# lucidrains/transfusion-pytorch

Hardware: NVIDIA H100
Metric: train tokens/sec (text+latent) at d=512 L=8 seq=1024 (higher is better)
Workload: dtype bf16

## Files before the change

### include/tfx_b200.h

```cpp
#ifndef TFX_B200_H
#define TFX_B200_H

#ifdef __cplusplus
extern "C" {
#endif

#define TFX_B200_VERSION 200

const char* tfx_last_error(void);
int tfx_version(void);
int tfx_init(int device);


int tfx_gemm_set_cluster_mode(int mode);

int tfx_gemm_store(const void* A, long long lda, int a_mn_major, const void* B, long long ldb, int b_mn_major, int M, int N, int K,
                   float* out_f32, long long ld_f32, void* out_bf16, long long ld_bf16, const float* bias, const long long* row_off,
                   float alpha, int accumulate, int k_splits, void* stream);

int tfx_gemm_qkvg(const void* u, long long ldu, const void* W, long long ldw, int M, int H, int D, void* q, void* k, void* v, float* gates, float* qk_inv,
                  const float* q_gamma, const float* k_gamma, const int* rope_pos, const float* rope_cs_t , int rope_len,
                  const int* kv_rows, float* mix_pre, void* stream);

int tfx_gemm_resid(const void* A, long long lda, const void* A2, long long lda2, int K1, const void* W, long long ldw, int M, int N, int K, const float* bias,
                   const float* x_res, float* x_out, void* x_out_bf16, void* y_bf16, const int* cond_row, const float* zgate, long long zgate_ld,
                   const float* layerscale, void* stream);

int tfx_gemm_geglu(const void* u, long long ldu, const void* W1p, long long ldw, const float* b1p, int M, int Np, int K, void* vg, void* h, void* stream);
int tfx_gemm_geglu_drop(const void* u, long long ldu, const void* W1p, long long ldw, const float* b1p, int M, int Np, int K, void* vg, void* h,
                        const void* drop_key , float p, int layer, void* stream);

int tfx_attn_fwd(const void* q, const void* k, const void* v, long long ld_q, long long ld_k, long long ld_v, const float* gates, int H,
                 const int* kv_limit, const int* tile_q0, const int* tile_qend, const int* tile_kv0, const int* tile_kvend, int n_tiles,
                 void* o, long long ld_o, float* lse, int M, float scale, float softcap, const float* skip_if_fast , void* stream);
int tfx_attn_fast_params(const float* q_gamma, const float* k_gamma, int dim_head, float scale, float softcap, float* params , void* stream);
int tfx_attn_fwd_tc(const void* q, const void* k, const void* v, long long ld_q, long long ld_k, long long ld_v, const float* gates, int H,
                    const int* kv_limit, const int* tile_q0, const int* tile_qend, const int* tile_kv0, const int* tile_kvend, int n_tiles,
// ... 106 lines not shown
```

### transfusion_pytorch_b200/_lib.py

```python
from __future__ import annotations

import ctypes
import os
from ctypes import c_void_p, c_int, c_longlong, c_ulonglong, c_float, c_char_p, POINTER

_HERE = os.path.dirname(os.path.abspath(__file__))
LIB_PATH = os.path.join(_HERE, 'libtfx_b200.so')

_lib = None

VP, I, LL, F, ULL = c_void_p, c_int, c_longlong, c_float, c_ulonglong

SIGNATURES = {
    'tfx_init': [I],
    'tfx_gemm_set_cluster_mode': [I],
    'tfx_gemm_store': [VP, LL, I, VP, LL, I, I, I, I, VP, LL, VP, LL, VP, VP, F, I, I, VP],
    'tfx_gemm_qkvg': [VP, LL, VP, LL, I, I, I, VP, VP, VP, VP, VP, VP, VP, VP, VP, I, VP, VP, VP],
    'tfx_gemm_resid': [VP, LL, VP, LL, I, VP, LL, I, I, I, VP, VP, VP, VP, VP, VP, VP, LL, VP, VP],
    'tfx_gemm_geglu': [VP, LL, VP, LL, VP, I, I, I, VP, VP, VP],
    'tfx_gemm_geglu_drop': [VP, LL, VP, LL, VP, I, I, I, VP, VP, VP, F, I, VP],
    'tfx_attn_fwd': [VP, VP, VP, LL, LL, LL, VP, I, VP, VP, VP, VP, VP, I, VP, LL, VP, I, F, F, VP, VP],
    'tfx_attn_fwd_tc': [VP, VP, VP, LL, LL, LL, VP, I, VP, VP, VP, VP, VP, I, VP, LL, VP, I, I, F, F, VP, VP],
    'tfx_attn_fast_params': [VP, VP, I, F, F, VP, VP],
    'tfx_attn_bwd_prep': [VP, VP, VP, VP, VP, VP, VP, I, I, VP],
    'tfx_attn_bwd': [VP, VP, VP, VP, LL, LL, LL, LL, VP, VP, VP, VP, VP, VP, VP, I, VP, VP, VP, LL, I, I, F, F, VP, VP],
    'tfx_attn_bwd_tc': [VP, VP, VP, VP, LL, LL, LL, LL, VP, VP, VP, VP, VP, VP, VP, VP, I, VP, VP, VP, LL, I, I, F, F, VP, VP],
    'tfx_qk_bwd_pack': [VP, VP, VP, VP, VP, VP, VP, VP, VP, VP, VP, VP, LL, VP, VP, I, I, VP],
    'tfx_adaln_fwd': [VP, VP, VP, LL, VP, VP, VP, I, I, VP],
    'tfx_adaln_bwd': [VP, VP, VP, VP, VP, LL, VP, VP, VP, LL, VP, I, I, VP],
    'tfx_resid_bwd': [VP, VP, VP, VP, LL, VP, VP, VP, LL, VP, VP, I, I, VP],
    'tfx_attn_residual_fwd': [VP, I, VP, VP, VP, VP, VP, I, I, VP],
    'tfx_attn_residual_bwd': [VP, VP, I, VP, VP, VP, VP, VP, VP, VP, VP, I, I, I, VP],
    'tfx_attn_residual_bwd2': [VP, I, I, VP, VP, VP, VP, I, VP, VP, VP, VP, VP, I, VP, VP, VP, I, I, VP],
    'tfx_attn_residual_fwd_h16': [VP, I, VP, VP, VP, VP, VP, I, I, VP],
    'tfx_attn_residual_bwd_h16': [VP, VP, I, VP, VP, VP, VP, VP, VP, VP, VP, I, I, I, VP],
    'tfx_rmsnorm_fwd': [VP, VP, VP, VP, VP, VP, I, I, VP],
    'tfx_rmsnorm_bwd': [VP, VP, VP, VP, VP, I, I, VP],
    'tfx_rep_cos_fwd_bwd': [VP, VP, I, VP, I, VP, VP, VP, VP, I, I, VP],
# ... 61 lines not shown
    lib.tfx_last_error.argtypes = []
    lib.tfx_version.restype = c_int
    lib.tfx_version.argtypes = []
    lib.tfx_geglu_bwd_rows_per_block.restype = c_int
    lib.tfx_geglu_bwd_rows_per_block.argtypes = []
    lib.tfx_attn_residual_bwd_workspace_floats.restype = c_longlong
    lib.tfx_attn_residual_bwd_workspace_floats.argtypes = [c_int, c_int]
    lib.tfx_rep_cos_blocks.restype = c_int
    lib.tfx_rep_cos_blocks.argtypes = [c_int]
    for name, argtypes in SIGNATURES.items():
        fn = getattr(lib, name)
        fn.argtypes = argtypes
        fn.restype = c_int
    _lib = lib
    return lib


def check(rc: int, name: str):
    if rc != 0:
        msg = _lib.tfx_last_error().decode(errors = 'replace') if _lib is not None else ''
        raise TfxError(f'{name} failed (code {rc}): {msg}')


class Ops:

    def __init__(self):
        self.lib = load()
        import torch
        self._torch = torch
        self.launches = 0
        self.timing = None
        self.order = None

    def stream(self):
        return self._torch.cuda.current_stream().cuda_stream

    def __getattr__(self, name):
        fn = getattr(self.lib, 'tfx_' + name)
        torch = self._torch

        def call(*args):
            conv = []
            for a in args:
                if a is None:
                    conv.append(None)
                elif torch.is_tensor(a):
# ... 20 lines not shown
```

### transfusion_pytorch_b200/csrc/gemm_api.cu

```cuda
#include "gemm_sm90.cuh"
#include "common.cuh"
#include "../../include/tfx_b200.h"
#include <string.h>

namespace tfx { int num_sms(); }
using namespace tfx;
#define ST(s) reinterpret_cast<cudaStream_t>(s)

static int finish(int rc, const char* what) {
  if (rc == 0) return 0;
  if (rc <= -1000) set_error("%s: cuTensorMapEncodeTiled failed (CUresult %d) - check 16-byte alignment of pointers and row pitches", what, -(rc + 1000));
  else if (rc == -1) set_error("%s: cuTensorMapEncodeTiled entry point unavailable (no CUDA driver?)", what);
  else if (rc == -2) set_error("%s: cudaFuncSetAttribute(max dynamic smem) failed: %s", what, cudaGetErrorString(cudaGetLastError()));
  else set_error("%s: kernel launch failed: %s", what, cudaGetErrorString(cudaGetLastError()));
  return rc;
}

static int dispatch_major(const GemmOperand& A, const GemmOperand& B, const GemmParams& p, cudaStream_t st) {
  const int sms = num_sms();
  if (!A.mn_major && !B.mn_major) return launch_gemm_t<false, false, EPI_STORE>(A, B, p, sms, st);
  if (!A.mn_major && B.mn_major) return launch_gemm_t<false, true, EPI_STORE>(A, B, p, sms, st);
  if (A.mn_major && B.mn_major) return launch_gemm_t<true, true, EPI_STORE>(A, B, p, sms, st);
  return launch_gemm_t<true, false, EPI_STORE>(A, B, p, sms, st);
}

extern "C" {

int tfx_gemm_set_cluster_mode(int mode) {
  TFX_REQUIRE(mode >= 1 && mode <= 3, "gemm_set_cluster_mode: mode %d not in {1 (never pair, default), 2 (always pair), 3 (pair long-K launches)}", mode);
  gemm_cluster_mode_ref() = mode;
  return 0;
}

int tfx_gemm_store(const void* A, long long lda, int a_mn_major, const void* B, long long ldb, int b_mn_major, int M, int N, int K,
                   float* out_f32, long long ld_f32, void* out_bf16, long long ld_bf16, const float* bias, const long long* row_off,
                   float alpha, int accumulate, int k_splits, void* stream) {
  if (M <= 0 || N <= 0) return 0;
  TFX_REQUIRE(K > 0, "gemm_store: K must be > 0");
  TFX_REQUIRE(lda % 8 == 0 && ldb % 8 == 0, "gemm_store: operand row pitches (%lld, %lld) must be multiples of 8 bf16", lda, ldb);
  TFX_REQUIRE(!(k_splits > 1) || (accumulate && out_f32 && !out_bf16 && !bias), "gemm_store: split-K requires fp32 accumulate output only");
  GemmParams p; memset(&p, 0, sizeof(p));
  p.M = M; p.N = N; p.K = K; p.k_splits = k_splits < 1 ? 1 : k_splits;
  p.out_f32 = out_f32; p.ld_f32 = ld_f32; p.out_bf16 = (__nv_bfloat16*)out_bf16; p.ld_bf16 = ld_bf16; p.bias = bias; p.row_off = row_off;
  p.alpha = alpha; p.accumulate_f32 = accumulate;
  GemmOperand a{A, lda, a_mn_major != 0}, b{B, ldb, b_mn_major != 0};
  const int rc = dispatch_major(a, b, p, ST(stream));
  return finish(rc, "gemm_store");
}

int tfx_gemm_qkvg(const void* u, long long ldu, const void* W, long long ldw, int M, int H, int D, void* q, void* k, void* v, float* gates, float* qk_inv,
                  const float* q_gamma, const float* k_gamma, const int* rope_pos, const float* rope_cs_t, int rope_len, const int* kv_rows, float* mix_pre, void* stream) {
  if (M <= 0) return 0;
  TFX_REQUIRE(!mix_pre || H <= 16, "gemm_qkvg: the value-residual mix columns share the 32-column gate slab: heads must be <= 16 (got %d)", H);
// ... 48 lines not shown
```

### transfusion_pytorch_b200/csrc/gemm_sm90.cuh

```cuda
#pragma once
#include "sm90_ptx.cuh"
#include "dropout.cuh"

namespace tfx {

constexpr int GEMM_BM = 128;
constexpr int GEMM_BN = 128;
constexpr int GEMM_BK = 64;
constexpr int GEMM_UK = 16;

enum : int { EPI_STORE = 0, EPI_QKVG = 1, EPI_RESID = 2, EPI_GEGLU = 3, EPI_GEGLU_DROP = 4 };

struct GemmParams {
  int M, N, K;
  int k_splits;
  float* out_f32; long long ld_f32;
  __nv_bfloat16* out_bf16; long long ld_bf16;
  const float* bias;
  const long long* row_off;
  float alpha;
  int accumulate_f32;
  int K1;
  int H;
  __nv_bfloat16 *q, *k, *v;
// ... 133 lines not shown
      *reinterpret_cast<uint4*>(g + row * pitch + ch * 16) = *reinterpret_cast<const uint4*>(sw + row * 64 + ((ch ^ ((row >> 1) & 3)) << 4));
  }
}

__device__ __forceinline__ void stg64_store_rows(const uint8_t* sw, int lane, uint8_t* g, long long pitch, int rows_valid, const int* __restrict__ rows) {
#pragma unroll
  for (int it = 0; it < 4; ++it) {
    const int row = it * 8 + (lane >> 2), ch = lane & 3;
    if (row < rows_valid)
      *reinterpret_cast<uint4*>(g + (long long)rows[row] * pitch + ch * 16) = *reinterpret_cast<const uint4*>(sw + row * 64 + ((ch ^ ((row >> 1) & 3)) << 4));
  }
}
template <int CH>
__device__ __forceinline__ void stg_store_rows(const uint8_t* sw, int lane, uint8_t* g, long long pitch, int rows_valid, const int* __restrict__ rows) {
  constexpr int RPI = 32 / CH;
#pragma unroll
  for (int it = 0; it < 32 / RPI; ++it) {
    const int row = it * RPI + lane / CH, ch = lane % CH;
    if (row < rows_valid)
      *reinterpret_cast<uint4*>(g + (long long)rows[row] * pitch + ch * 16) = *reinterpret_cast<const uint4*>(sw + row * 128 + ((ch ^ (row & 7)) << 4));
  }
}

template <bool A_MN, bool B_MN, int EPI, int CL>
__global__ void __launch_bounds__(384, 1)
gemm_sm90_kernel(const __grid_constant__ CUtensorMap tmA, const __grid_constant__ CUtensorMap tmA2, const __grid_constant__ CUtensorMap tmB, const GemmParams p) {
  using Cfg = GemmCfg<EPI>;
  constexpr bool GEGLU = EPI == EPI_GEGLU || EPI == EPI_GEGLU_DROP;
  constexpr int BN = GEMM_BN;
  constexpr int STAGES = Cfg::STAGES;
  static_assert(Cfg::STAGE_BYTES % 1024 == 0 && 2 * STAGES <= 32, "stage alignment / barrier area");
  extern __shared__ __align__(1024) uint8_t smem_raw[];
  uint8_t* smem = smem_raw;
  if (threadIdx.x == 0 && (smem_u32(smem) & 1023u) != 0) __trap();
  uint8_t* acc = smem + STAGES * Cfg::STAGE_BYTES;
  uint8_t* staging = acc + Cfg::ACC_BYTES;
  uint64_t* bars = reinterpret_cast<uint64_t*>(staging + Cfg::STAGING);
  uint64_t* full_bar = bars;
  uint64_t* empty_bar = bars + STAGES;

  const int warp = threadIdx.x >> 5, lane = threadIdx.x & 31;
  const int m_tiles = (p.M + GEMM_BM - 1) / GEMM_BM;
  const int n_tiles = (p.N + BN - 1) / BN;
  const int kb_total = (p.K + GEMM_BK - 1) / GEMM_BK;
  const int kb_per_split = (kb_total + p.k_splits - 1) / p.k_splits;
  const int m_units = (m_tiles + CL - 1) / CL;
// ... 119 lines not shown
      {
        const int r0 = quad * 16 + (lane >> 2);
#pragma unroll
        for (int q = 0; q < 16; ++q) {
          const int c = 8 * q + 2 * (lane & 3);
          *reinterpret_cast<float2*>(acc + acc_off(r0, c)) = make_float2(d0[4 * q], d0[4 * q + 1]);
          *reinterpret_cast<float2*>(acc + acc_off(r0 + 8, c)) = make_float2(d0[4 * q + 2], d0[4 * q + 3]);
          *reinterpret_cast<float2*>(acc + acc_off(r0 + 64, c)) = make_float2(d1[4 * q], d1[4 * q + 1]);
          *reinterpret_cast<float2*>(acc + acc_off(r0 + 72, c)) = make_float2(d1[4 * q + 2], d1[4 * q + 3]);
        }
      }
      named_bar_sync(BAR_TILE + cw, 128);

      const int wrow0 = m_blk * GEMM_BM + quad * 32;
      const int row = wrow0 + lane;
      const bool row_ok = row < p.M;
      const int rows_valid = min(32, p.M - wrow0);
      const int col0 = n_blk * BN;
      int qk_pos = 0;
      if constexpr (EPI == EPI_QKVG) { qk_pos = row_ok ? p.rope_pos[row] : 0; }
      if constexpr (EPI == EPI_RESID) { qk_pos = (row_ok && p.cond_row) ? p.cond_row[row] : -1; }

      if constexpr (EPI == EPI_STORE) {
        const bool f32_staged = p.out_f32 && (p.row_off || (p.ld_f32 & 3) == 0) && ((reinterpret_cast<uintptr_t>(p.out_f32) & 15) == 0);
        const bool bf16_staged = p.out_bf16 && (p.ld_bf16 & 7) == 0 && ((reinterpret_cast<uintptr_t>(p.out_bf16) & 15) == 0);
#pragma unroll 1
        for (int c = 0; c < BN / 32; ++c) {
          const int cbase = col0 + c * 32;
          if (cbase >= p.N) break;
          uint32_t r[32];
          acc_ld32(acc, erow, c * 32, r);
          const bool full = cbase + 32 <= p.N;
          float v[32];
#pragma unroll
          for (int j = 0; j < 32; ++j) v[j] = __uint_as_float(r[j]);
          if (p.alpha != 1.f) {
#pragma unroll
            for (int j = 0; j < 32; ++j) v[j] *= p.alpha;
          }
          if (p.bias) {
            if (full) {
#pragma unroll
              for (int j = 0; j < 32; j += 4) { const float4 b = *reinterpret_cast<const float4*>(p.bias + cbase + j); v[j] += b.x; v[j + 1] += b.y; v[j + 2] += b.z; v[j + 3] += b.w; }
            } else {
              for (int j = 0; j < 32; ++j) if (cbase + j < p.N) v[j] += p.bias[cbase + j];
            }
          }
          if (p.out_f32) {
            if (full && f32_staged) {
#pragma unroll
              for (int j = 0; j < 32; ++j) r[j] = __float_as_uint(v[j]);
              stg_put<8>(sw, lane, r);
              __syncwarp();
#pragma unroll
              for (int it = 0; it < 8; ++it) {
                const int rr = it * 4 + (lane >> 3), ch = lane & 7;
                if (rr < rows_valid) {
                  const long long off = p.row_off ? p.row_off[wrow0 + rr] : (long long)(wrow0 + rr) * p.ld_f32;
                  if (off >= 0) {
                    float* dst = p.out_f32 + off + cbase + ch * 4;
                    const float4 t = *reinterpret_cast<const float4*>(sw + rr * 128 + ((ch ^ (rr & 7)) << 4));
                    if ((reinterpret_cast<uintptr_t>(dst) & 15) == 0) {
                      if (p.accumulate_f32) asm volatile("red.global.add.v4.f32 [%0], {%1, %2, %3, %4};" ::"l"(dst), "f"(t.x), "f"(t.y), "f"(t.z), "f"(t.w) : "memory");
                      else *reinterpret_cast<float4*>(dst) = t;
                    } else {
                      if (p.accumulate_f32) { atomicAdd(dst, t.x); atomicAdd(dst + 1, t.y); atomicAdd(dst + 2, t.z); atomicAdd(dst + 3, t.w); }
                      else { dst[0] = t.x; dst[1] = t.y; dst[2] = t.z; dst[3] = t.w; }
                    }
                  }
                }
              }
              __syncwarp();
            } else if (row_ok) {
              const long long off = p.row_off ? p.row_off[row] : (long long)row * p.ld_f32;
              if (off >= 0) {
                float* dst = p.out_f32 + off + cbase;
                for (int j = 0; j < 32; ++j)
                  if (cbase + j < p.N) { if (p.accumulate_f32) atomicAdd(dst + j, v[j]); else dst[j] = v[j]; }
              }
            }
          }
          if (p.out_bf16) {
            if (full && bf16_staged) {
              uint32_t w[16];
#pragma unroll
              for (int j = 0; j < 16; ++j) w[j] = pack_bf16(v[2 * j], v[2 * j + 1]);
              stg_put<4>(sw, lane, w);
              __syncwarp();
              stg_store<4>(sw, lane, reinterpret_cast<uint8_t*>(p.out_bf16 + (long long)wrow0 * p.ld_bf16 + cbase), p.ld_bf16 * 2, rows_valid);
              __syncwarp();
            } else if (row_ok) {
              __nv_bfloat16* dst = p.out_bf16 + (long long)row * p.ld_bf16 + cbase;
              for (int j = 0; j < 32; ++j) if (cbase + j < p.N) dst[j] = __float2bfloat16(v[j]);
            }
          }
        }
      } else if constexpr (EPI == EPI_QKVG) {
        const int tps = p.H >> 1;
        const int kind = n_blk / tps;
        const int tis = n_blk - kind * tps;
        const long long HI = (long long)p.H * 64;
        if (kind <= 1) {
          const float* gamma = kind == 0 ? p.q_gamma : p.k_gamma;
          __nv_bfloat16* dstm = kind == 0 ? p.q : p.k;
          const float2* cs = p.rope_cs + qk_pos;
#pragma unroll
          for (int hh = 0; hh < 2; ++hh) {
            uint32_t r0[32], r1[32];
            acc_ld32(acc, erow, hh * 64, r0);
            acc_ld32(acc, erow, hh * 64 + 32, r1);
            float ss = 0.f;
#pragma unroll
            for (int j = 0; j < 32; ++j) { float a = __uint_as_float(r0[j]), b = __uint_as_float(r1[j]); ss += a * a + b * b; }
            const float inv = 1.f / fmaxf(sqrtf(ss), 1e-12f);
            const int head = tis * 2 + hh;
            if (row_ok) p.qk_inv[(long long)row * 2 * p.H + kind * p.H + head] = inv;
            const float sc = inv * 8.f;
            uint32_t outw[32];
// ... 152 lines not shown
            const float2 o = geglu_pair(make_float2(g[j], g[j + 1]), make_float2(v[j], v[j + 1]));
            g[j] = o.x; g[j + 1] = o.y;
          }
          if constexpr (EPI == EPI_GEGLU_DROP) {
#pragma unroll
            for (int j = 0; j < 32; ++j) g[j] = (keep[c] >> j) & 1u ? g[j] * p.drop.scale : 0.f;
          }
          __syncwarp();
          stg64_put_pack(sw, lane, g);
          __syncwarp();
          stg64_store(sw, lane, reinterpret_cast<uint8_t*>(p.h + (long long)wrow0 * (p.N / 2) + n_blk * 64 + c * 32), (long long)p.N, rows_valid);
          __syncwarp();
        }
      }
      if (!GEGLU && has_next) named_bar_arrive(BAR_ACC + (cw ^ 1), 256);
    }
  }
  if constexpr (CL > 1) {
    __syncthreads();
    cluster_sync_all();
  }
}

typedef CUresult (*PFN_encodeTiled)(CUtensorMap*, CUtensorMapDataType, cuuint32_t, void*, const cuuint64_t*, const cuuint64_t*,
                                    const cuuint32_t*, const cuuint32_t*, CUtensorMapInterleave, CUtensorMapSwizzle,
                                    CUtensorMapL2promotion, CUtensorMapFloatOOBfill);

inline PFN_encodeTiled get_encode_fn() {
  static PFN_encodeTiled fn = nullptr;
  if (!fn) {
    void* f = nullptr;
    cudaDriverEntryPointQueryResult qres;
    if (cudaGetDriverEntryPoint("cuTensorMapEncodeTiled", &f, cudaEnableDefault, &qres) != cudaSuccess || !f) return nullptr;
    fn = reinterpret_cast<PFN_encodeTiled>(f);
  }
  return fn;
}

inline int make_tmap_bf16(CUtensorMap* tm, const void* ptr, long long inner, long long outer, long long ld, int box_rows) {
  PFN_encodeTiled enc = get_encode_fn();
  if (!enc) return -1;
  cuuint64_t dims[2] = {(cuuint64_t)inner, (cuuint64_t)outer};
  cuuint64_t strides[1] = {(cuuint64_t)ld * 2};
  cuuint32_t box[2] = {64, (cuuint32_t)box_rows};
  cuuint32_t estr[2] = {1, 1};
  CUresult r = enc(tm, CU_TENSOR_MAP_DATA_TYPE_BFLOAT16, 2, const_cast<void*>(ptr), dims, strides, box, estr,
                   CU_TENSOR_MAP_INTERLEAVE_NONE, CU_TENSOR_MAP_SWIZZLE_128B, CU_TENSOR_MAP_L2_PROMOTION_L2_256B,
                   CU_TENSOR_MAP_FLOAT_OOB_FILL_NONE);
  return r == CUDA_SUCCESS ? 0 : -(int)r - 1000;
}

struct GemmOperand {
  const void* ptr;
  long long ld;
  bool mn_major;
  const void* ptr2 = nullptr;
  long long ld2 = 0;
};

inline int& gemm_cluster_mode_ref() {
  static int mode = -1;
  if (mode < 0) { const char* e = getenv("TFX_GEMM_CLUSTER"); mode = e ? atoi(e) : 1; }
  return mode;
}

template <bool A_MN, bool B_MN, int EPI>
int launch_gemm_t(const GemmOperand& A, const GemmOperand& B, const GemmParams& p_in, int num_sms, cudaStream_t stream) {
  using Cfg = GemmCfg<EPI>;
  GemmParams p = p_in;
  CUtensorMap tmA, tmA2, tmB;
  int rc;
  const bool two = (!A_MN) && A.ptr2 != nullptr;
  if (!two) p.K1 = p.K;
  if (!A_MN) rc = make_tmap_bf16(&tmA, A.ptr, two ? p.K1 : p.K, p.M, A.ld, GEMM_BM); else rc = make_tmap_bf16(&tmA, A.ptr, p.M, p.K, A.ld, GEMM_BK);
  if (rc) return rc;
  if (two) { rc = make_tmap_bf16(&tmA2, A.ptr2, p.K - p.K1, p.M, A.ld2, GEMM_BM); if (rc) return rc; } else tmA2 = tmA;
  {
    const int kbt = (p.K + GEMM_BK - 1) / GEMM_BK;
    if (p.k_splits < 1) p.k_splits = 1;
    if (p.k_splits > kbt) p.k_splits = kbt;
    const int per = (kbt + p.k_splits - 1) / p.k_splits;
    p.k_splits = (kbt + per - 1) / per;
  }
  const int m_tiles = (p.M + GEMM_BM - 1) / GEMM_BM, n_tiles = (p.N + GEMM_BN - 1) / GEMM_BN;
  const int items = m_tiles * n_tiles * p.k_splits;
  if (items <= 0) return 0;
  const int mode = gemm_cluster_mode_ref();
  const int kb_item = ((p.K + GEMM_BK - 1) / GEMM_BK + p.k_splits - 1) / p.k_splits;
  const bool paired = mode == 2 || (mode == 3 && m_tiles >= 2 && kb_item >= 16 && items >= 2 * num_sms);
  if (!B_MN) rc = make_tmap_bf16(&tmB, B.ptr, p.K, p.N, B.ld, paired ? GEMM_BN / 2 : GEMM_BN); else rc = make_tmap_bf16(&tmB, B.ptr, p.N, p.K, B.ld, GEMM_BK);
  if (rc) return rc;
  if (paired) {
    auto kern = gemm_sm90_kernel<A_MN, B_MN, EPI, 2>;
    static int max_clusters = 0;
    cudaLaunchConfig_t cfg;
    memset(&cfg, 0, sizeof(cfg));
    cudaLaunchAttribute at[1];
    at[0].id = cudaLaunchAttributeClusterDimension;
    at[0].val.clusterDim.x = 2; at[0].val.clusterDim.y = 1; at[0].val.clusterDim.z = 1;
    cfg.blockDim = dim3(Cfg::THREADS); cfg.dynamicSmemBytes = Cfg::SMEM_BYTES; cfg.stream = stream; cfg.attrs = at; cfg.numAttrs = 1;
    if (!max_clusters) {
      if (cudaFuncSetAttribute(kern, cudaFuncAttributeMaxDynamicSharedMemorySize, Cfg::SMEM_BYTES) != cudaSuccess) return -2;
      cfg.gridDim = dim3(2 * (num_sms / 2));
      int nc = 0;
      if (cudaOccupancyMaxActiveClusters(&nc, kern, &cfg) != cudaSuccess || nc < 1) { cudaGetLastError(); nc = num_sms / 2; }
      max_clusters = nc < num_sms / 2 ? nc : num_sms / 2;
    }
    const int pair_items = ((m_tiles + 1) / 2) * n_tiles * p.k_splits;
    const int clusters = pair_items < max_clusters ? pair_items : max_clusters;
    cfg.gridDim = dim3(2 * clusters);
    return cudaLaunchKernelEx(&cfg, kern, tmA, tmA2, tmB, p) == cudaSuccess ? 0 : -3;
// ... 14 lines not shown
```

### transfusion_pytorch_b200/engine.py

```python
from __future__ import annotations

import math
import os
import ctypes
from dataclasses import dataclass

import numpy as np
import torch
from torch import Tensor

from . import _lib
from ._pinned import POOL
from .modality_processing import RaggedBatch

BF16, F32, I32, I64 = torch.bfloat16, torch.float32, torch.int32, torch.int64


def _round_up(x: int, m: int) -> int:
    return (x + m - 1) // m * m


_EMPTY_I32 = np.zeros(0, dtype = np.int32)


# ... 30 lines not shown
    tab = np.zeros(len(jobs), dtype = dt)
    blk_job, blk_first = [], []
    for j, (src, ld_src, c_src, row_src, d, r_dst, c_dst, f32) in enumerate(jobs):
        tab[j] = (src.data_ptr(), ld_src, row_src.data_ptr() if row_src is not None else 0, d.data_ptr(), r_dst, c_src, c_dst, f32, 0)
        nb = (r_dst * c_dst + 2047) // 2048
        blk_first.append(len(blk_job))
        blk_job.extend([j] * nb)
    return (torch.from_numpy(tab.view(np.uint8).copy()).to(device), torch.tensor(blk_job, dtype = I32, device = device),
            torch.tensor(blk_first, dtype = I32, device = device), len(blk_job))


def w1_row_src(inner: int) -> np.ndarray:
    Ip = _round_up(inner, 64)
    src = np.full(2 * Ip, -1, dtype = np.int64)
    for t in range(Ip // 64):
        for j in range(64):
            c = 64 * t + j
            if c < inner:
                src[128 * t + j] = c
                src[128 * t + 64 + j] = inner + c
    return src


def wgrad_splits(n_out, n_in, K, sms, ks):
    tiles = ((n_out + 127) // 128) * ((n_in + 255) // 256 if (n_in % 256 == 0 or n_in >= 1024) else (n_in + 127) // 128)
    best, best_eff = 1, 0.0
    for s in range(1, 65):
        if K // s < 1024 and s > 1:
            break
        items = tiles * s
        eff = items / (-(-items // sms) * sms)
        if eff > best_eff + 0.02 or (abs(eff - best_eff) <= 0.02 and s <= ks and s > best):
            best, best_eff = s, eff
    return best


class KVCache:

    def __init__(self, engine, n_slabs: int, cap: int):
        self.n_slabs, self.cap, self.rows = int(n_slabs), int(cap), int(n_slabs) * int(cap)
        nbytes = 2 * engine.depth * self.rows * engine.HI * 2
        assert nbytes < 96 << 30, f'kv cache of {nbytes / 2**30:.1f} GiB requested ({n_slabs} slabs x {cap} rows): lower max_length / batch the prompts'
        self.k = torch.zeros(engine.depth, self.rows, engine.HI, device = engine.device, dtype = BF16)
        self.v = torch.zeros(engine.depth, self.rows, engine.HI, device = engine.device, dtype = BF16)
        self.vl = torch.zeros_like(self.v) if engine.laser else None

    def slab_start(self, s):
        return np.asarray(s, dtype = np.int64) * self.cap


class Engine:
    def __init__(self, model):
        self.ops = _lib.Ops()
        self.model = model
        tr = model.transformer
        self.D, self.H, self.depth = tr.dim, tr.heads, tr.depth
        self.HI = self.H * 64
# ... 563 lines not shown
        st = self.state
        assert st['train'], 'backward() needs a train forward'
        rep_at = None
        if g_rep is not None:
            rep_at = st.get('rep_layer')
            assert rep_at is not None and g_rep.dtype == F32 and g_rep.is_contiguous() and g_rep.shape == (st['rb'].M, self.D), 'g_rep: fp32 [M, D] of a rep_layer forward'
        self._prepare_grads()
        self._grads_clean = False
        self._dirty = True
        if gscale is not None:
            gs = gscale.detach().float().reshape(1)
            self.ops.scale_bf16(st['dlogits'], gs, st['dlogits'].numel())
            for dp in st['dpred']:
                if dp is not None:
                    self.ops.scale_bf16(dp, gs, dp.numel())
        rb, dv = st['rb'], st['rb'].dev
        o, D, HI, H, Ip, M, inner = self.ops, self.D, self.HI, self.H, self.Ip, st['rb'].M, self.inner
        pk, nc, S = self.packed, rb.n_cond, rb.S
        cond_row = dv['cond_row'] if nc > 0 else None
        tab_ld, zg_ld = self.W * 3 * D, self.W * D
        ks = max(1, min(64, M // 2048))
        sms = torch.cuda.get_device_properties(self.device).multi_processor_count
        def ksplit(n_out, n_in, K = M):
            return wgrad_splits(n_out, n_in, K, sms, ks)
        def wgrad(dy, ld_dy, n_out, act, ld_act, n_in, gname, K = M):
            o.gemm_store(dy, ld_dy, 1, act, ld_act, 1, n_out, n_in, K, self.G(gname), n_in, None, 0, None, None, 1.0, 1, ksplit(n_out, n_in, K))

        dlog = st['dlogits']
        d_out = self.buf('d_out', (M, D), F32)
        o.gemm_store(dlog, self.Vp, 0, pk['wvocab'], D, 1, M, D, self.V, d_out, D, None, 0, None, None, 1.0, 0, 1)
        wgrad(dlog, self.Vp, self.V, st['outb'], D, D, 'to_text_logits.weight')
        if S > 0:
            dmod = self.buf('dmod', (S, D), F32)
            any_flow = False
            for t, (s0, s1) in enumerate(rb.type_rows):
                n = s1 - s0
                dp = st['dpred'][t] if n else None
                if dp is None:
                    if n:
                        dmod[s0:s1].zero_()
                    continue
                any_flow = True
                dl, dlp = self.dls[t], self.dlp[t]
                o.gemm_store(dp, dlp, 0, pk[f'wm2l{t}'], D, 1, n, D, dl, dmod[s0:s1], D, None, 0, None, None, 1.0, 0, 1)
                wgrad(dp, dlp, dl, st['omod'][s0:s1], D, D, f'model_to_latent_projs.{t}.weight', K = n)
            dneg = None
            if any_flow and self.clean:
# ... 242 lines not shown
        a = eng.buf('rh_a', (M, D), F32)
        o.gemm_store(h, Ip, 0, self.w2p, Ip, 0, M, D, Ip, a, D, None, 0, b2, None, 1.0, 0, 1)
        da = eng.buf('rh_da', (M, D), BF16)
        part = eng.buf('rh_part', (int(o.lib.tfx_rep_cos_blocks(M)),), torch.float64)
        ticket = eng.buf('rh_ticket', (1,), I32, zero = True)
        loss = eng.buf('rh_loss', (1,), F32)
        o.rep_cos_fwd_bwd(a, teacher, 1 if teacher.dtype == BF16 else 0, g, M, da, part, ticket, loss, M, D)
        self.state = dict(x = x, u = u, vg = vg, h = h, da = da, g = g, M = M)
        return loss[0].clone()

    def backward(self, g_loss: Tensor | None = None) -> Tensor:
        eng, o, st = self.eng, self.eng.ops, self.state
        M, D, inner, Ip = st['M'], self.D, self.inner, self.Ip
        head = self.head
        params = [head[0].gamma, head[1].net[0].weight, head[1].net[0].bias, head[1].net[3].weight, head[1].net[3].bias]
        for p in params:
            if p.grad is None:
                p.grad = torch.zeros_like(p)
        ggamma, gw1, gb1, gw2, gb2 = (p.grad for p in params)
        da = st['da']
        if g_loss is not None:
            o.scale_bf16(da, (g_loss.detach().float().reshape(1) / st['g']), da.numel())
        sms = torch.cuda.get_device_properties(eng.device).multi_processor_count
        ks = max(1, min(64, M // 2048))
        dh = eng.buf('rh_dh', (M, Ip), BF16)
        o.gemm_store(da, D, 0, self.w2p, Ip, 1, M, Ip, D, None, 0, dh, Ip, None, None, 1.0, 0, 1)
        o.gemm_store(da, D, 1, st['h'], Ip, 1, D, inner, M, gw2, 0, None, 0, None, self.w2_rows, 1.0, 1, wgrad_splits(D, inner, M, sms, ks))
        o.colsum_bf16(da, D, M, D, None, gb2)
        dvg = eng.buf('rh_dvg', (M, 2 * Ip), BF16)
        rpb = o.lib.tfx_geglu_bwd_rows_per_block()
        nblk = (M + rpb - 1) // rpb
        part = eng.buf('rh_geglu_part', (nblk, 2 * Ip), F32)
        o.geglu_bwd(dh, st['vg'], dvg, M, Ip, None, None, part)
        o.colsum_f32(part, 2 * Ip, nblk, 2 * Ip, self.b1_cols, gb1)
        du = eng.buf('rh_du', (M, D), F32)
        o.gemm_store(dvg, 2 * Ip, 0, self.w1p, D, 1, M, D, 2 * Ip, du, D, None, 0, None, None, 1.0, 0, 1)
        o.gemm_store(dvg, 2 * Ip, 1, st['u'], D, 1, 2 * Ip, D, M, gw1, 0, None, 0, None, self.w1_rows, 1.0, 1, wgrad_splits(2 * Ip, D, M, sms, ks))
        gx = eng.buf('rh_gx', (M, D), F32)
        o.rmsnorm_bwd(du, st['x'], head[0].gamma, gx, ggamma, M, D)
        return gx
```

Before: 1.186 million.

## Add 256-row wide GEMM kernel for long-K store launches and cost-based split choice

Adds a second warp-specialized sm90 GEMM kernel using 256x128 tiles, where each consumer warpgroup issues two m64n128 wgmma per k-step. It is used for gemm_store calls whose per-item K length is at least 16 blocks, mainly the weight-gradient GEMMs. The intent is more reuse of B tiles and fewer items per tile. The k-split heuristic now queries the library for item geometry and picks the smallest split within 5% of a wave-quantized cost estimate, and it is cached. The shared store epilogue is factored into a helper, and misaligned f32 rows now take a realigned vector path. The trade-offs are fewer resident work items, which risks worse wave balance, and more register pressure from 128 accumulators per thread.

New measurement: 1.222 million, median of 6. 1.03x the previous value.

```diff
diff --git a/include/tfx_b200.h b/include/tfx_b200.h
--- a/include/tfx_b200.h
+++ b/include/tfx_b200.h
@@ -13,6 +13,10 @@
 
 
 int tfx_gemm_set_cluster_mode(int mode);
+
+int tfx_gemm_set_wide_mode(int mode);
+
+int tfx_gemm_store_items(int M, int N, int K, int a_mn_major, int b_mn_major, int k_splits, int* geometry);
 
 int tfx_gemm_store(const void* A, long long lda, int a_mn_major, const void* B, long long ldb, int b_mn_major, int M, int N, int K,
                    float* out_f32, long long ld_f32, void* out_bf16, long long ld_bf16, const float* bias, const long long* row_off,
diff --git a/transfusion_pytorch_b200/_lib.py b/transfusion_pytorch_b200/_lib.py
--- a/transfusion_pytorch_b200/_lib.py
+++ b/transfusion_pytorch_b200/_lib.py
@@ -14,6 +14,8 @@
 SIGNATURES = {
     'tfx_init': [I],
     'tfx_gemm_set_cluster_mode': [I],
+    'tfx_gemm_set_wide_mode': [I],
+    'tfx_gemm_store_items': [I, I, I, I, I, I, VP],
     'tfx_gemm_store': [VP, LL, I, VP, LL, I, I, I, I, VP, LL, VP, LL, VP, VP, F, I, I, VP],
     'tfx_gemm_qkvg': [VP, LL, VP, LL, I, I, I, VP, VP, VP, VP, VP, VP, VP, VP, VP, I, VP, VP, VP],
     'tfx_gemm_resid': [VP, LL, VP, LL, I, VP, LL, I, I, I, VP, VP, VP, VP, VP, VP, VP, LL, VP, VP],
@@ -121,6 +123,13 @@
         raise TfxError(f'{name} failed (code {rc}): {msg}')
 
 
+def gemm_store_items(M: int, N: int, K: int, a_mn: int, b_mn: int, k_splits: int):
+    lib = load()
+    geo = (c_int * 4)()
+    check(lib.tfx_gemm_store_items(M, N, K, a_mn, b_mn, k_splits, geo), 'tfx_gemm_store_items')
+    return tuple(geo)
+
+
 class Ops:
 
     def __init__(self):
diff --git a/transfusion_pytorch_b200/csrc/gemm_api.cu b/transfusion_pytorch_b200/csrc/gemm_api.cu
--- a/transfusion_pytorch_b200/csrc/gemm_api.cu
+++ b/transfusion_pytorch_b200/csrc/gemm_api.cu
@@ -18,6 +18,12 @@
 
 static int dispatch_major(const GemmOperand& A, const GemmOperand& B, const GemmParams& p, cudaStream_t st) {
   const int sms = num_sms();
+  if (gemm_store_wide(p.K, p.k_splits)) {
+    if (!A.mn_major && !B.mn_major) return launch_gemm_wide_t<false, false>(A, B, p, sms, st);
+    if (!A.mn_major && B.mn_major) return launch_gemm_wide_t<false, true>(A, B, p, sms, st);
+    if (A.mn_major && B.mn_major) return launch_gemm_wide_t<true, true>(A, B, p, sms, st);
+    return launch_gemm_wide_t<true, false>(A, B, p, sms, st);
+  }
   if (!A.mn_major && !B.mn_major) return launch_gemm_t<false, false, EPI_STORE>(A, B, p, sms, st);
   if (!A.mn_major && B.mn_major) return launch_gemm_t<false, true, EPI_STORE>(A, B, p, sms, st);
   if (A.mn_major && B.mn_major) return launch_gemm_t<true, true, EPI_STORE>(A, B, p, sms, st);
@@ -29,6 +35,24 @@
 int tfx_gemm_set_cluster_mode(int mode) {
   TFX_REQUIRE(mode >= 1 && mode <= 3, "gemm_set_cluster_mode: mode %d not in {1 (never pair, default), 2 (always pair), 3 (pair long-K launches)}", mode);
   gemm_cluster_mode_ref() = mode;
+  return 0;
+}
+
+int tfx_gemm_set_wide_mode(int mode) {
+  TFX_REQUIRE(mode >= 1 && mode <= 3, "gemm_set_wide_mode: mode %d not in {1 (long work items, default), 2 (always), 3 (never)}", mode);
+  gemm_wide_mode_ref() = mode;
+  return 0;
+}
+
+int tfx_gemm_store_items(int M, int N, int K, int a_mn_major, int b_mn_major, int k_splits, int* geometry) {
+  TFX_REQUIRE(M > 0 && N > 0 && K > 0 && geometry, "gemm_store_items: needs M, N, K > 0 (got %d, %d, %d) and an output array", M, N, K);
+  (void)a_mn_major; (void)b_mn_major;
+  const int tile_m = gemm_store_wide(K, k_splits) ? GemmWideCfg::BM : GEMM_BM;
+  const int s = gemm_effective_splits(K, k_splits);
+  geometry[0] = ((M + tile_m - 1) / tile_m) * ((N + GEMM_BN - 1) / GEMM_BN) * s;
+  geometry[1] = gemm_kb_per_item(K, s);
+  geometry[2] = tile_m;
+  geometry[3] = s;
   return 0;
 }
 
diff --git a/transfusion_pytorch_b200/csrc/gemm_sm90.cuh b/transfusion_pytorch_b200/csrc/gemm_sm90.cuh
--- a/transfusion_pytorch_b200/csrc/gemm_sm90.cuh
+++ b/transfusion_pytorch_b200/csrc/gemm_sm90.cuh
@@ -179,6 +179,99 @@
   }
 }
 
+template <class RowOf>
+__device__ __forceinline__ void store_slice(const GemmParams& p, uint8_t* sw, int lane, uint32_t (&r)[32], int cbase, RowOf row_of) {
+  const bool f32_staged = p.out_f32 && (p.row_off || (p.ld_f32 & 3) == 0) && ((reinterpret_cast<uintptr_t>(p.out_f32) & 15) == 0);
+  const bool bf16_staged = p.out_bf16 && (p.ld_bf16 & 7) == 0 && ((reinterpret_cast<uintptr_t>(p.out_bf16) & 15) == 0);
+  const int row = row_of(lane);
+  const bool row_ok = row < p.M;
+  const bool full = cbase + 32 <= p.N;
+  float v[32];
+#pragma unroll
+  for (int j = 0; j < 32; ++j) v[j] = __uint_as_float(r[j]);
+  if (p.alpha != 1.f) {
+#pragma unroll
+    for (int j = 0; j < 32; ++j) v[j] *= p.alpha;
+  }
+  if (p.bias) {
+    if (full) {
+#pragma unroll
+      for (int j = 0; j < 32; j += 4) { const float4 b = *reinterpret_cast<const float4*>(p.bias + cbase + j); v[j] += b.x; v[j + 1] += b.y; v[j + 2] += b.z; v[j + 3] += b.w; }
+    } else {
+      for (int j = 0; j < 32; ++j) if (cbase + j < p.N) v[j] += p.bias[cbase + j];
+    }
+  }
+  if (p.out_f32) {
+    if (full && f32_staged) {
+#pragma unroll
+      for (int j = 0; j < 32; ++j) r[j] = __float_as_uint(v[j]);
+      stg_put<8>(sw, lane, r);
+      __syncwarp();
+      auto put = [&](float* dst, float x) { if (p.accumulate_f32) atomicAdd(dst, x); else *dst = x; };
+#pragma unroll
+      for (int it = 0; it < 8; ++it) {
+        const int rr = it * 4 + (lane >> 3), ch = lane & 7;
+        const int grow = row_of(rr);
+        if (grow < p.M) {
+          const long long off = p.row_off ? p.row_off[grow] : (long long)grow * p.ld_f32;
+          if (off >= 0) {
+            float* drow = p.out_f32 + off + cbase;
+            const uint8_t* srow = sw + rr * 128;
+            const int a = (int)(reinterpret_cast<uintptr_t>(drow) >> 2) & 3;
+            if (a == 0) {
+              float* dst = drow + ch * 4;
+              const float4 t = *reinterpret_cast<const float4*>(srow + ((ch ^ (rr & 7)) << 4));
+              if (p.accumulate_f32) asm volatile("red.global.add.v4.f32 [%0], {%1, %2, %3, %4};" ::"l"(dst), "f"(t.x), "f"(t.y), "f"(t.z), "f"(t.w) : "memory");
+              else *reinterpret_cast<float4*>(dst) = t;
+            } else {
+              const int pe = 4 - a;
+              auto col = [&](int j) { return *reinterpret_cast<const float*>(srow + (((j >> 2) ^ (rr & 7)) << 4) + (j & 3) * 4); };
+              if (ch < 7) {
+                const int j = pe + 4 * ch;
+                float* dst = drow + j;
+                const float4 t = make_float4(col(j), col(j + 1), col(j + 2), col(j + 3));
+                if (p.accumulate_f32) asm volatile("red.global.add.v4.f32 [%0], {%1, %2, %3, %4};" ::"l"(dst), "f"(t.x), "f"(t.y), "f"(t.z), "f"(t.w) : "memory");
+                else *reinterpret_cast<float4*>(dst) = t;
+              } else {
+#pragma unroll
+                for (int i = 0; i < 4; ++i) { const int j = i < pe ? i : 28 + i; put(drow + j, col(j)); }
+              }
+            }
+          }
+        }
+      }
+      __syncwarp();
+    } else if (row_ok) {
+      const long long off = p.row_off ? p.row_off[row] : (long long)row * p.ld_f32;
+      if (off >= 0) {
+        float* dst = p.out_f32 + off + cbase;
+        for (int j = 0; j < 32; ++j)
+          if (cbase + j < p.N) { if (p.accumulate_f32) atomicAdd(dst + j, v[j]); else dst[j] = v[j]; }
+      }
+    }
+  }
+  if (p.out_bf16) {
+    if (full && bf16_staged) {
+      uint32_t w[16];
+#pragma unroll
+      for (int j = 0; j < 16; ++j) w[j] = pack_bf16(v[2 * j], v[2 * j + 1]);
+      stg_put<4>(sw, lane, w);
+      __syncwarp();
+#pragma unroll
+      for (int it = 0; it < 4; ++it) {
+        const int rr = it * 8 + (lane >> 2), ch = lane & 3;
+        const int grow = row_of(rr);
+        if (grow < p.M)
+          *reinterpret_cast<uint4*>(p.out_bf16 + (long long)grow * p.ld_bf16 + cbase + ch * 8) = *reinterpret_cast<const uint4*>(sw + rr * 128 + ((ch ^ (rr & 7)) << 4));
+      }
+      __syncwarp();
+    } else if (row_ok) {
+      __nv_bfloat16* dst = p.out_bf16 + (long long)row * p.ld_bf16 + cbase;
+      for (int j = 0; j < 32; ++j) if (cbase + j < p.N) dst[j] = __float2bfloat16(v[j]);
+    }
+  }
+}
+
 template <bool A_MN, bool B_MN, int EPI, int CL>
 __global__ void __launch_bounds__(384, 1)
 gemm_sm90_kernel(const __grid_constant__ CUtensorMap tmA, const __grid_constant__ CUtensorMap tmA2, const __grid_constant__ CUtensorMap tmB, const GemmParams p) {
@@ -344,78 +437,13 @@
       if constexpr (EPI == EPI_RESID) { qk_pos = (row_ok && p.cond_row) ? p.cond_row[row] : -1; }
 
       if constexpr (EPI == EPI_STORE) {
-        const bool f32_staged = p.out_f32 && (p.row_off || (p.ld_f32 & 3) == 0) && ((reinterpret_cast<uintptr_t>(p.out_f32) & 15) == 0);
-        const bool bf16_staged = p.out_bf16 && (p.ld_bf16 & 7) == 0 && ((reinterpret_cast<uintptr_t>(p.out_bf16) & 15) == 0);
 #pragma unroll 1
         for (int c = 0; c < BN / 32; ++c) {
           const int cbase = col0 + c * 32;
           if (cbase >= p.N) break;
           uint32_t r[32];
           acc_ld32(acc, erow, c * 32, r);
-          const bool full = cbase + 32 <= p.N;
-          float v[32];
-#pragma unroll
-          for (int j = 0; j < 32; ++j) v[j] = __uint_as_float(r[j]);
-          if (p.alpha != 1.f) {
-#pragma unroll
-            for (int j = 0; j < 32; ++j) v[j] *= p.alpha;
-          }
-          if (p.bias) {
-            if (full) {
-#pragma unroll
-              for (int j = 0; j < 32; j += 4) { const float4 b = *reinterpret_cast<const float4*>(p.bias + cbase + j); v[j] += b.x; v[j + 1] += b.y; v[j + 2] += b.z; v[j + 3] += b.w; }
-            } else {
-              for (int j = 0; j < 32; ++j) if (cbase + j < p.N) v[j] += p.bias[cbase + j];
-            }
-          }
-          if (p.out_f32) {
-            if (full && f32_staged) {
-#pragma unroll
-              for (int j = 0; j < 32; ++j) r[j] = __float_as_uint(v[j]);
-              stg_put<8>(sw, lane, r);
-              __syncwarp();
-#pragma unroll
-              for (int it = 0; it < 8; ++it) {
-                const int rr = it * 4 + (lane >> 3), ch = lane & 7;
-                if (rr < rows_valid) {
-                  const long long off = p.row_off ? p.row_off[wrow0 + rr] : (long long)(wrow0 + rr) * p.ld_f32;
-                  if (off >= 0) {
-                    float* dst = p.out_f32 + off + cbase + ch * 4;
-                    const float4 t = *reinterpret_cast<const float4*>(sw + rr * 128 + ((ch ^ (rr & 7)) << 4));
-                    if ((reinterpret_cast<uintptr_t>(dst) & 15) == 0) {
-                      if (p.accumulate_f32) asm volatile("red.global.add.v4.f32 [%0], {%1, %2, %3, %4};" ::"l"(dst), "f"(t.x), "f"(t.y), "f"(t.z), "f"(t.w) : "memory");
-                      else *reinterpret_cast<float4*>(dst) = t;
-                    } else {
-                      if (p.accumulate_f32) { atomicAdd(dst, t.x); atomicAdd(dst + 1, t.y); atomicAdd(dst + 2, t.z); atomicAdd(dst + 3, t.w); }
-                      else { dst[0] = t.x; dst[1] = t.y; dst[2] = t.z; dst[3] = t.w; }
-                    }
-                  }
-                }
-              }
-              __syncwarp();
-            } else if (row_ok) {
-              const long long off = p.row_off ? p.row_off[row] : (long long)row * p.ld_f32;
-              if (off >= 0) {
-                float* dst = p.out_f32 + off + cbase;
-                for (int j = 0; j < 32; ++j)
-                  if (cbase + j < p.N) { if (p.accumulate_f32) atomicAdd(dst + j, v[j]); else dst[j] = v[j]; }
-              }
-            }
-          }
-          if (p.out_bf16) {
-            if (full && bf16_staged) {
-              uint32_t w[16];
-#pragma unroll
-              for (int j = 0; j < 16; ++j) w[j] = pack_bf16(v[2 * j], v[2 * j + 1]);
-              stg_put<4>(sw, lane, w);
-              __syncwarp();
-              stg_store<4>(sw, lane, reinterpret_cast<uint8_t*>(p.out_bf16 + (long long)wrow0 * p.ld_bf16 + cbase), p.ld_bf16 * 2, rows_valid);
-              __syncwarp();
-            } else if (row_ok) {
-              __nv_bfloat16* dst = p.out_bf16 + (long long)row * p.ld_bf16 + cbase;
-              for (int j = 0; j < 32; ++j) if (cbase + j < p.N) dst[j] = __float2bfloat16(v[j]);
-            }
-          }
+          store_slice(p, sw, lane, r, cbase, [&](int i) { return wrow0 + i; });
         }
       } else if constexpr (EPI == EPI_QKVG) {
         const int tps = p.H >> 1;
@@ -614,6 +642,155 @@
   }
 }
 
+struct GemmWideCfg {
+  static constexpr int BM = 256;
+  static constexpr int THREADS = 384;
+  static constexpr int STAGES = 4;
+  static constexpr int A_BYTES = BM * GEMM_BK * 2;
+  static constexpr int B_BYTES = GEMM_BN * GEMM_BK * 2;
+  static constexpr int STAGE_BYTES = A_BYTES + B_BYTES;
+  static constexpr int STAGING = 8 * 4096;
+  static constexpr int SMEM_BYTES = STAGES * STAGE_BYTES + STAGING + 1024  + 256 ;
+  static_assert(SMEM_BYTES <= 227 * 1024, "shared memory of one block");
+};
+
+template <bool A_MN, bool B_MN>
+__global__ void __launch_bounds__(384, 1)
+gemm_sm90_wide_kernel(const __grid_constant__ CUtensorMap tmA, const __grid_constant__ CUtensorMap tmB, const GemmParams p) {
+  using Cfg = GemmWideCfg;
+  constexpr int BM = Cfg::BM, BN = GEMM_BN, STAGES = Cfg::STAGES;
+  static_assert(Cfg::STAGE_BYTES % 1024 == 0, "stage alignment");
+  extern __shared__ __align__(1024) uint8_t smem_raw[];
+  uint8_t* smem = smem_raw;
+  if (threadIdx.x == 0 && (smem_u32(smem) & 1023u) != 0) __trap();
+  uint8_t* staging = smem + STAGES * Cfg::STAGE_BYTES;
+  uint64_t* full_bar = reinterpret_cast<uint64_t*>(staging + Cfg::STAGING);
+  uint64_t* empty_bar = full_bar + STAGES;
+
+  const int warp = threadIdx.x >> 5, lane = threadIdx.x & 31;
+  const int m_tiles = (p.M + BM - 1) / BM;
+  const int n_tiles = (p.N + BN - 1) / BN;
+  const int kb_total = (p.K + GEMM_BK - 1) / GEMM_BK;
+  const int kb_per_split = (kb_total + p.k_splits - 1) / p.k_splits;
+  const int tiles = m_tiles * n_tiles;
+  const int num_items = tiles * p.k_splits;
+
+  if (threadIdx.x == 0) {
+    tma_prefetch_desc(&tmA);
+    tma_prefetch_desc(&tmB);
+    for (int s = 0; s < STAGES; ++s) { mbar_init(&full_bar[s], 1); mbar_init(&empty_bar[s], 8); }
+    mbar_fence_init();
+  }
+  __syncthreads();
+
+  if (warp < 4) {
+    setmaxnreg_dec<40>();
+    if (threadIdx.x == 0) {
+      int stage = 0; uint32_t phase = 0;
+      for (int item = blockIdx.x; item < num_items; item += gridDim.x) {
+        const int split = item / tiles;
+        const int rem = item - split * tiles;
+        const int m_blk = rem / n_tiles, n_blk = rem - m_blk * n_tiles;
+        const int kb0 = split * kb_per_split;
+        const int kb1 = min(kb0 + kb_per_split, kb_total);
+        for (int kb = kb0; kb < kb1; ++kb) {
+          mbar_wait(&empty_bar[stage], phase ^ 1);
+          uint8_t* sA = smem + stage * Cfg::STAGE_BYTES;
+          uint8_t* sB = sA + Cfg::A_BYTES;
+          mbar_expect_tx(&full_bar[stage], Cfg::STAGE_BYTES);
+          if (!A_MN) {
+            tma_load_2d(&tmA, &full_bar[stage], sA, kb * GEMM_BK, m_blk * BM);
+          } else {
+#pragma unroll
+            for (int a = 0; a < BM / 64; ++a)
+              tma_load_2d(&tmA, &full_bar[stage], sA + a * (GEMM_BK * 128), m_blk * BM + a * 64, kb * GEMM_BK);
+          }
+          if (!B_MN) {
+            tma_load_2d(&tmB, &full_bar[stage], sB, kb * GEMM_BK, n_blk * BN);
+          } else {
+#pragma unroll
+            for (int a = 0; a < BN / 64; ++a)
+              tma_load_2d(&tmB, &full_bar[stage], sB + a * (GEMM_BK * 128), n_blk * BN + a * 64, kb * GEMM_BK);
+          }
+          if (++stage == STAGES) { stage = 0; phase ^= 1; }
+        }
+      }
+    }
+  } else {
+    setmaxnreg_inc<232>();
+    const int cw = (warp >> 2) - 1;
+    const int quad = warp & 3;
+    uint8_t* sw = staging + (4 * cw + quad) * 4096;
+    const uint32_t a_half = (uint32_t)cw * (A_MN ? 2 * GEMM_BK * 128 : 128 * 128);
+    int stage = 0; uint32_t phase = 0;
+    auto release = [&](int s) { __syncwarp(); if (lane == 0) mbar_arrive(&empty_bar[s]); };
+    for (int item = blockIdx.x; item < num_items; item += gridDim.x) {
+      const int split = item / tiles;
+      const int rem = item - split * tiles;
+      const int m_blk = rem / n_tiles, n_blk = rem - m_blk * n_tiles;
+      const int kb0 = split * kb_per_split;
+      const int kb1 = min(kb0 + kb_per_split, kb_total);
+      float d0[64], d1[64];
+#pragma unroll
+      for (int i = 0; i < 64; ++i) { d0[i] = 0.f; d1[i] = 0.f; }
+      int prev_stage = -1;
+      for (int kb = kb0; kb < kb1; ++kb) {
+        mbar_wait(&full_bar[stage], phase);
+        const uint32_t sA = smem_u32(smem + stage * Cfg::STAGE_BYTES) + a_half;
+        const uint32_t sB = smem_u32(smem + stage * Cfg::STAGE_BYTES) + Cfg::A_BYTES;
+        wgmma_reg_fence(d0);
+        wgmma_reg_fence(d1);
+        wgmma_fence();
+#pragma unroll
+        for (int k = 0; k < GEMM_BK / GEMM_UK; ++k) {
+          const uint64_t db = B_MN ? wgmma_desc_sw128(sB + k * (GEMM_UK * 128), GEMM_BK * 128, 1024)
+                                   : wgmma_desc_sw128(sB + k * (GEMM_UK * 2), 16, 1024);
+          const uint64_t da0 = A_MN ? wgmma_desc_sw128(sA + k * (GEMM_UK * 128), GEMM_BK * 128, 1024)
+                                    : wgmma_desc_sw128(sA + k * (GEMM_UK * 2), 16, 1024);
+          const uint64_t da1 = A_MN ? wgmma_desc_sw128(sA + GEMM_BK * 128 + k * (GEMM_UK * 128), GEMM_BK * 128, 1024)
+                                    : wgmma_desc_sw128(sA + 64 * 128 + k * (GEMM_UK * 2), 16, 1024);
+          const uint32_t acc_flag = (kb > kb0 || k > 0) ? 1u : 0u;
+          wgmma_m64n128_ss<A_MN ? 1 : 0, B_MN ? 1 : 0>(d0, da0, db, acc_flag);
+          wgmma_m64n128_ss<A_MN ? 1 : 0, B_MN ? 1 : 0>(d1, da1, db, acc_flag);
+        }
+        wgmma_commit();
+        wgmma_wait<1>();
+        if (prev_stage >= 0) release(prev_stage);
+        prev_stage = stage;
+        if (++stage == STAGES) { stage = 0; phase ^= 1; }
+      }
+      wgmma_wait<0>();
+      wgmma_reg_fence(d0);
+      wgmma_reg_fence(d1);
+      if (prev_stage >= 0) release(prev_stage);
+
+      const int wrow0 = m_blk * BM + 128 * cw + 16 * quad;
+      const int r0 = lane >> 2;
+#pragma unroll
+      for (int c = 0; c < BN / 32; ++c) {
+        const int cbase = n_blk * BN + c * 32;
+        if (cbase >= p.N) break;
+#pragma unroll
+        for (int q4 = 0; q4 < 4; ++q4) {
+          const int q = 4 * c + q4, col = 8 * q4 + 2 * (lane & 3);
+          auto put2 = [&](int rr, float x, float y) {
+            *reinterpret_cast<float2*>(sw + rr * 128 + ((((col >> 2) ^ (rr & 7))) << 4) + (col & 3) * 4) = make_float2(x, y);
+          };
+          put2(r0, d0[4 * q], d0[4 * q + 1]);
+          put2(r0 + 8, d0[4 * q + 2], d0[4 * q + 3]);
+          put2(r0 + 16, d1[4 * q], d1[4 * q + 1]);
+          put2(r0 + 24, d1[4 * q + 2], d1[4 * q + 3]);
+        }
+        __syncwarp();
+        uint32_t r[32];
+        stg_get<8>(sw, lane, r);
+        __syncwarp();
+        store_slice(p, sw, lane, r, cbase, [&](int i) { return wrow0 + (i & 15) + ((i >> 4) << 6); });
+      }
+    }
+  }
+}
+
 typedef CUresult (*PFN_encodeTiled)(CUtensorMap*, CUtensorMapDataType, cuuint32_t, void*, const cuuint64_t*, const cuuint64_t*,
                                     const cuuint32_t*, const cuuint32_t*, CUtensorMapInterleave, CUtensorMapSwizzle,
                                     CUtensorMapL2promotion, CUtensorMapFloatOOBfill);
@@ -656,6 +833,46 @@
   return mode;
 }
 
+inline int gemm_effective_splits(int K, int k_splits) {
+  const int kbt = (K + GEMM_BK - 1) / GEMM_BK;
+  int s = k_splits < 1 ? 1 : k_splits > kbt ? kbt : k_splits;
+  const int per = (kbt + s - 1) / s;
+  return (kbt + per - 1) / per;
+}
+inline int gemm_kb_per_item(int K, int k_splits) { return ((K + GEMM_BK - 1) / GEMM_BK + k_splits - 1) / k_splits; }
+
+constexpr int GEMM_WIDE_MIN_KB = 16;
+inline int& gemm_wide_mode_ref() { static int mode = 1; return mode; }
+inline bool gemm_store_wide(int K, int k_splits) {
+  const int mode = gemm_wide_mode_ref();
+  if (mode != 1) return mode == 2;
+  return gemm_cluster_mode_ref() == 1 && gemm_kb_per_item(K, gemm_effective_splits(K, k_splits)) >= GEMM_WIDE_MIN_KB;
+}
+
+template <bool A_MN, bool B_MN>
+int launch_gemm_wide_t(const GemmOperand& A, const GemmOperand& B, const GemmParams& p_in, int num_sms, cudaStream_t stream) {
+  using Cfg = GemmWideCfg;
+  GemmParams p = p_in;
+  p.K1 = p.K;
+  p.k_splits = gemm_effective_splits(p.K, p.k_splits);
+  const int items = ((p.M + Cfg::BM - 1) / Cfg::BM) * ((p.N + GEMM_BN - 1) / GEMM_BN) * p.k_splits;
+  if (items <= 0) return 0;
+  CUtensorMap tmA, tmB;
+  int rc = !A_MN ? make_tmap_bf16(&tmA, A.ptr, p.K, p.M, A.ld, Cfg::BM) : make_tmap_bf16(&tmA, A.ptr, p.M, p.K, A.ld, GEMM_BK);
+  if (rc) return rc;
+  rc = !B_MN ? make_tmap_bf16(&tmB, B.ptr, p.K, p.N, B.ld, GEMM_BN) : make_tmap_bf16(&tmB, B.ptr, p.N, p.K, B.ld, GEMM_BK);
+  if (rc) return rc;
+  auto kern = gemm_sm90_wide_kernel<A_MN, B_MN>;
+  static bool attr_set = false;
+  if (!attr_set) {
+    if (cudaFuncSetAttribute(kern, cudaFuncAttributeMaxDynamicSharedMemorySize, Cfg::SMEM_BYTES) != cudaSuccess) return -2;
+    attr_set = true;
+  }
+  const int grid = items < num_sms ? items : num_sms;
+  kern<<<grid, Cfg::THREADS, Cfg::SMEM_BYTES, stream>>>(tmA, tmB, p);
+  return cudaGetLastError() == cudaSuccess ? 0 : -3;
+}
+
 template <bool A_MN, bool B_MN, int EPI>
 int launch_gemm_t(const GemmOperand& A, const GemmOperand& B, const GemmParams& p_in, int num_sms, cudaStream_t stream) {
   using Cfg = GemmCfg<EPI>;
@@ -667,18 +884,12 @@
   if (!A_MN) rc = make_tmap_bf16(&tmA, A.ptr, two ? p.K1 : p.K, p.M, A.ld, GEMM_BM); else rc = make_tmap_bf16(&tmA, A.ptr, p.M, p.K, A.ld, GEMM_BK);
   if (rc) return rc;
   if (two) { rc = make_tmap_bf16(&tmA2, A.ptr2, p.K - p.K1, p.M, A.ld2, GEMM_BM); if (rc) return rc; } else tmA2 = tmA;
-  {
-    const int kbt = (p.K + GEMM_BK - 1) / GEMM_BK;
-    if (p.k_splits < 1) p.k_splits = 1;
-    if (p.k_splits > kbt) p.k_splits = kbt;
-    const int per = (kbt + p.k_splits - 1) / p.k_splits;
-    p.k_splits = (kbt + per - 1) / per;
-  }
+  p.k_splits = gemm_effective_splits(p.K, p.k_splits);
   const int m_tiles = (p.M + GEMM_BM - 1) / GEMM_BM, n_tiles = (p.N + GEMM_BN - 1) / GEMM_BN;
   const int items = m_tiles * n_tiles * p.k_splits;
   if (items <= 0) return 0;
   const int mode = gemm_cluster_mode_ref();
-  const int kb_item = ((p.K + GEMM_BK - 1) / GEMM_BK + p.k_splits - 1) / p.k_splits;
+  const int kb_item = gemm_kb_per_item(p.K, p.k_splits);
   const bool paired = mode == 2 || (mode == 3 && m_tiles >= 2 && kb_item >= 16 && items >= 2 * num_sms);
   if (!B_MN) rc = make_tmap_bf16(&tmB, B.ptr, p.K, p.N, B.ld, paired ? GEMM_BN / 2 : GEMM_BN); else rc = make_tmap_bf16(&tmB, B.ptr, p.N, p.K, B.ld, GEMM_BK);
   if (rc) return rc;
diff --git a/transfusion_pytorch_b200/engine.py b/transfusion_pytorch_b200/engine.py
--- a/transfusion_pytorch_b200/engine.py
+++ b/transfusion_pytorch_b200/engine.py
@@ -1,5 +1,6 @@
 from __future__ import annotations
 
+import functools
 import math
 import os
 import ctypes
@@ -76,17 +77,16 @@
     return src
 
 
-def wgrad_splits(n_out, n_in, K, sms, ks):
-    tiles = ((n_out + 127) // 128) * ((n_in + 255) // 256 if (n_in % 256 == 0 or n_in >= 1024) else (n_in + 127) // 128)
-    best, best_eff = 1, 0.0
+@functools.lru_cache(maxsize = None)
+def wgrad_splits(n_out, n_in, K, sms):
+    cost = {}
     for s in range(1, 65):
-        if K // s < 1024 and s > 1:
+        items, kb, tile_m, s_eff = _lib.gemm_store_items(n_out, n_in, K, 1, 1, s)
+        if s_eff != s or (s > 1 and kb < 16):
             break
-        items = tiles * s
-        eff = items / (-(-items // sms) * sms)
-        if eff > best_eff + 0.02 or (abs(eff - best_eff) <= 0.02 and s <= ks and s > best):
-            best, best_eff = s, eff
-    return best
+        cost[s] = -(-items // sms) * kb * tile_m // 128
+    best = min(cost.values())
+    return min(s for s, c in cost.items() if c <= 1.05 * best)
 
 
 class KVCache:
@@ -696,7 +696,7 @@
         ks = max(1, min(64, M // 2048))
         sms = torch.cuda.get_device_properties(self.device).multi_processor_count
         def ksplit(n_out, n_in, K = M):
-            return wgrad_splits(n_out, n_in, K, sms, ks)
+            return wgrad_splits(n_out, n_in, K, sms)
         def wgrad(dy, ld_dy, n_out, act, ld_act, n_in, gname, K = M):
             o.gemm_store(dy, ld_dy, 1, act, ld_act, 1, n_out, n_in, K, self.G(gname), n_in, None, 0, None, None, 1.0, 1, ksplit(n_out, n_in, K))
 
@@ -985,10 +985,9 @@
         if g_loss is not None:
             o.scale_bf16(da, (g_loss.detach().float().reshape(1) / st['g']), da.numel())
         sms = torch.cuda.get_device_properties(eng.device).multi_processor_count
-        ks = max(1, min(64, M // 2048))
         dh = eng.buf('rh_dh', (M, Ip), BF16)
         o.gemm_store(da, D, 0, self.w2p, Ip, 1, M, Ip, D, None, 0, dh, Ip, None, None, 1.0, 0, 1)
-        o.gemm_store(da, D, 1, st['h'], Ip, 1, D, inner, M, gw2, 0, None, 0, None, self.w2_rows, 1.0, 1, wgrad_splits(D, inner, M, sms, ks))
+        o.gemm_store(da, D, 1, st['h'], Ip, 1, D, inner, M, gw2, 0, None, 0, None, self.w2_rows, 1.0, 1, wgrad_splits(D, inner, M, sms))
         o.colsum_bf16(da, D, M, D, None, gb2)
         dvg = eng.buf('rh_dvg', (M, 2 * Ip), BF16)
         rpb = o.lib.tfx_geglu_bwd_rows_per_block()
@@ -998,7 +997,7 @@
         o.colsum_f32(part, 2 * Ip, nblk, 2 * Ip, self.b1_cols, gb1)
         du = eng.buf('rh_du', (M, D), F32)
         o.gemm_store(dvg, 2 * Ip, 0, self.w1p, D, 1, M, D, 2 * Ip, du, D, None, 0, None, None, 1.0, 0, 1)
-        o.gemm_store(dvg, 2 * Ip, 1, st['u'], D, 1, 2 * Ip, D, M, gw1, 0, None, 0, None, self.w1_rows, 1.0, 1, wgrad_splits(2 * Ip, D, M, sms, ks))
+        o.gemm_store(dvg, 2 * Ip, 1, st['u'], D, 1, 2 * Ip, D, M, gw1, 0, None, 0, None, self.w1_rows, 1.0, 1, wgrad_splits(2 * Ip, D, M, sms))
         gx = eng.buf('rh_gx', (M, D), F32)
         o.rmsnorm_bwd(du, st['x'], head[0].gamma, gx, ggamma, M, D)
         return gx
```
